# AliBahri94/GM3D

Hardware: AMD Instinct MI355X
Metric: point-clouds/sec pretrain step (N=1024,G=64) (higher is better)
Workload: dtype bf16

## Files before the change

### gm3d_amd/csrc/gemm_ws.hip

```cpp
#include "mfma.hpp"

namespace gm3d {

__device__ __forceinline__ void ws_wait_vm(int n) {
#define GM3D_WS_CASE(N_) case N_: asm volatile("s_waitcnt vmcnt(%0)" ::"n"(N_) : "memory"); break;
    switch (n) {
        GM3D_WS_CASE(0) GM3D_WS_CASE(4) GM3D_WS_CASE(8) GM3D_WS_CASE(12) GM3D_WS_CASE(16) GM3D_WS_CASE(24) GM3D_WS_CASE(32)
        GM3D_WS_CASE(36) GM3D_WS_CASE(48)
        default: asm volatile("s_waitcnt vmcnt(0)" ::: "memory"); break;
    }
#undef GM3D_WS_CASE
}

struct WsBn {
    const bf16_t* T;
    const float* scale;
    const float* shift;
    float* partial;
    int ldt;
    float slope;
};

constexpr int ws_depth(int ppl, int tile, int stage) {
    int d = 48 / ppl < 4 ? 48 / ppl : 4;
    while (d > 1 && (d + 1) * tile + stage > 152 * 1024) --d;
    return d;
}

template <int KT, int NW, int NL, int EPI, int TM>
__global__ __launch_bounds__(64 * (NW + NL)) void gemm_tn_ws_kernel(const bf16_t* __restrict__ A, const bf16_t* __restrict__ W,
                                                                     const float* __restrict__ bias, bf16_t* __restrict__ C, int M, int N,
                                                                     int lda, int ldw, int ldc, int tiles_n, bf16_t* __restrict__ P,
                                                                     uint8_t* __restrict__ ARG, int ldp, int bias_after_pool, WsBn bn,
                                                                     int Kreal, int pool16) {
    extern __shared__ __attribute__((aligned(16))) unsigned char wsm[];
    constexpr int BN = 32 * NW, NIMG = BN / 64 > 0 ? (BN + 63) / 64 : 1;
    constexpr int HALF = KT * 4096;
    constexpr int TILE = TM * HALF;
    constexpr int NP = TM * 4 * KT;
    constexpr int PPL = NP / NL;
    constexpr int STAGE = TM * NIMG * 4096;
    constexpr int DEPTH = ws_depth(PPL, TILE, STAGE);
    constexpr int NT = DEPTH + 1;
    static_assert(NP % NL == 0 && PPL <= 48, "loader split");
    unsigned char* stage = wsm + NT * TILE;
    const int tid = threadIdx.x, lane = tid & 63, w = __builtin_amdgcn_readfirstlane(tid >> 6);
    const int r = lane & 31, hh = lane >> 5;
    const int logical = xcd_tile(blockIdx.x, gridDim.x);
    const int tile_n = logical % tiles_n, first = logical / tiles_n, stride = gridDim.x / tiles_n;
    const int tiles_m = (M + 32 * TM - 1) / (32 * TM);
    const int nmine = first < tiles_m ? (tiles_m - first + stride - 1) / stride : 0;
    const int n0 = tile_n * BN;
    const unsigned lds0 = lds_addr(wsm);

    if (w >= NW) {
        const int lw = w - NW, prow = lane >> 3, pslot = lane & 7;
        auto issue = [&](int i) {
            const int m0 = (first + i * stride) * (32 * TM);
            const unsigned base = lds0 + (i % NT) * TILE;
#pragma unroll
            for (int q = 0; q < PPL; ++q) {
                const int p = lw * PPL + q, t = p / (4 * KT), pp = p - t * (4 * KT), kt = pp >> 2, row = 8 * (pp & 3) + prow;
                const int gr = m0 + 32 * t + row;
                const int am = gr < M ? gr : M - 1;
                int col = 64 * kt + ((pslot ^ swz(row)) << 3);
                col = col < Kreal ? col : 0;
                glds16(A + (size_t)am * lda + col, base + 1024 * p);
            }
        };
        for (int d = 0; d < DEPTH && d < nmine; ++d) issue(d);
        for (int i = 0; i < nmine; ++i) {
            if (i + DEPTH < nmine) issue(i + DEPTH);
            const int ahead = nmine - 1 - i < DEPTH ? nmine - 1 - i : DEPTH;
            ws_wait_vm(ahead * PPL);
            __builtin_amdgcn_s_barrier();
            __builtin_amdgcn_s_barrier();
        }
        return;
    }

    bf16x8 wreg[KT][4];
    {
        const bf16_t* wp = W + (size_t)(n0 + 32 * w + r) * ldw + 8 * hh;
#pragma unroll
        for (int kt = 0; kt < KT; ++kt)
#pragma unroll
            for (int s = 0; s < 4; ++s) {
                if (64 * kt + 16 * s + 8 * hh < Kreal) wreg[kt][s] = *reinterpret_cast<const bf16x8*>(wp + 64 * kt + 16 * s);
                else
#pragma unroll
                    for (int e = 0; e < 8; ++e) wreg[kt][s][e] = (bf16_t)0.0f;
            }
    }
    float bq[4][4];
#pragma unroll
    for (int q = 0; q < 4; ++q)
#pragma unroll
        for (int e = 0; e < 4; ++e) bq[q][e] = (EPI != 3 && bias) ? bias[n0 + 32 * w + 8 * q + 4 * hh + e] : 0.f;
    const float bcol = (EPI == 3 && bias) ? bias[n0 + 32 * w + r] : 0.f;
    const bool bias_in_tile = EPI != 3 || !bias_after_pool;
    float bn_a[4][4], bn_b[4][4];
    if (EPI == 4 || EPI == 5) {
#pragma unroll
        for (int q = 0; q < 4; ++q)
#pragma unroll
            for (int e = 0; e < 4; ++e) {
                const int col = n0 + 32 * w + 8 * q + 4 * hh + e;
                bn_a[q][e] = EPI == 4 ? bn.scale[col] : 0.f;
                bn_b[q][e] = EPI == 4 ? bn.shift[col] : 0.f;
            }
    }
    constexpr int CTHREADS = 64 * NW;

    for (int i = 0; i < nmine; ++i) {
        const int m0 = (first + i * stride) * (32 * TM);
        float tq[TM][4][4];
        if (EPI == 4 || EPI == 5) {
            typedef const __attribute__((address_space(4))) unsigned int* sptr_t;
#pragma unroll
            for (int t = 0; t < TM; ++t) {
                const size_t trow = pool16 ? (size_t)2 * ((m0 >> 5) + t) : (size_t)((m0 >> 5) + t);
                sptr_t tp = (sptr_t)(const void*)(bn.T + trow * bn.ldt + n0 + 32 * w);
                unsigned tw[16];
#pragma unroll
                for (int j = 0; j < 16; ++j) tw[j] = tp[j];
                if (pool16) {
                    sptr_t tp2 = (sptr_t)(const void*)(bn.T + (trow + 1) * bn.ldt + n0 + 32 * w);
                    unsigned tw2[16];
#pragma unroll
                    for (int j = 0; j < 16; ++j) tw2[j] = tp2[j];
                    if (r & 16) {
#pragma unroll
                        for (int j = 0; j < 16; ++j) tw[j] = tw2[j];
                    }
                }
#pragma unroll
                for (int q = 0; q < 4; ++q)
#pragma unroll
                    for (int e2 = 0; e2 < 2; ++e2) {
                        const unsigned u = hh ? tw[4 * q + 2 + e2] : tw[4 * q + e2];
                        tq[t][q][2 * e2] = __builtin_bit_cast(float, u << 16);
                        tq[t][q][2 * e2 + 1] = __builtin_bit_cast(float, u & 0xffff0000u);
                    }
            }
        }
        __builtin_amdgcn_s_barrier();
        const unsigned char* as = wsm + (i % NT) * TILE;
        f32x16 acc[TM];
#pragma unroll
        for (int t = 0; t < TM; ++t)
#pragma unroll
            for (int g = 0; g < 16; ++g) acc[t][g] = 0.f;
#pragma unroll
        for (int kt = 0; kt < KT; ++kt) {
            bf16x8 fa[TM][4];
#pragma unroll
            for (int t = 0; t < TM; ++t)
#pragma unroll
                for (int s = 0; s < 4; ++s) fa[t][s] = *reinterpret_cast<const bf16x8*>(as + t * HALF + kt * 4096 + swz_off(r, 2 * s + hh));
#pragma unroll
            for (int s = 0; s < 4; ++s)
#pragma unroll
                for (int t = 0; t < TM; ++t)
                    acc[t] = EPI == 3 ? mfma_bf16(fa[t][s], wreg[kt][s], acc[t])
                                      : mfma_bf16(wreg[kt][s], fa[t][s], acc[t]);
        }
        if (EPI == 3 && !C) __builtin_amdgcn_s_barrier();
        if (EPI == 3) {
            unsigned short rowbits[TM][16];
#pragma unroll
            for (int t = 0; t < TM; ++t) {
                unsigned best = 0, best2 = 0;
#pragma unroll
                for (int g = 0; g < 16; ++g) {
                    const bf16_t o = (bf16_t)(acc[t][g] + (bias_in_tile ? bcol : 0.f));
                    rowbits[t][g] = __builtin_bit_cast(unsigned short, o);
                    unsigned u = (unsigned)rowbits[t][g] << 16;
                    u = u == 0x80000000u ? 0u : u;
                    const unsigned k = (u ^ (unsigned)(((int)u >> 31) | (int)0x80000000)) & 0xffff0000u;
                    const unsigned key = k | (unsigned)(31 - (8 * (g >> 2) + 4 * hh + (g & 3)));
                    if (pool16 && g >= 8) best2 = key > best2 ? key : best2;
                    else best = key > best ? key : best;
                }
                {
                    const unsigned other = (unsigned)__shfl_xor((int)best, 32);
                    best = other > best ? other : best;
                    const unsigned other2 = (unsigned)__shfl_xor((int)best2, 32);
                    best2 = other2 > best2 ? other2 : best2;
                }
                if (hh == 0 && m0 + 32 * t < M) {
                    const unsigned k = best & 0xffff0000u;
                    const unsigned u = (k & 0x80000000u) ? (k & 0x7fff0000u) : (~k & 0xffff0000u);
                    float v = __builtin_bit_cast(float, u);
                    if (bias_after_pool) v += bcol;
                    if (!pool16) {
                        const size_t o = (size_t)((m0 >> 5) + t) * ldp + n0 + 32 * w + r;
                        P[o] = (bf16_t)v;
                        ARG[o] = (uint8_t)(31u - (best & 0xffu));
                    } else {
                        const size_t o = (size_t)((m0 >> 4) + 2 * t) * ldp + n0 + 32 * w + r;
                        P[o] = (bf16_t)v;
                        ARG[o] = (uint8_t)(31u - (best & 0xffu));
                        if (m0 + 32 * t + 16 < M) {
                            const unsigned k2 = best2 & 0xffff0000u;
                            const unsigned u2 = (k2 & 0x80000000u) ? (k2 & 0x7fff0000u) : (~k2 & 0xffff0000u);
                            float v2 = __builtin_bit_cast(float, u2);
                            if (bias_after_pool) v2 += bcol;
                            P[o + ldp] = (bf16_t)v2;
                            ARG[o + ldp] = (uint8_t)(15u - (best2 & 0xffu));
                        }
                    }
                }
            }
            if (!C) continue;
            const int ch = (((32 * w) & 63) + r) >> 3, sub = 2 * (r & 7);
#pragma unroll
            for (int t = 0; t < TM; ++t) {
                unsigned char* img = stage + (t * NIMG + ((32 * w) >> 6)) * 4096;
#pragma unroll
                for (int g = 0; g < 16; ++g) {
                    const int row = 8 * (g >> 2) + 4 * hh + (g & 3);
                    *reinterpret_cast<unsigned short*>(img + swz_off(row, ch) + sub) = rowbits[t][g];
                }
            }
        } else {
            const int cbase = ((32 * w) & 63) >> 3;
#pragma unroll
            for (int t = 0; t < TM; ++t) {
                unsigned char* img = stage + (t * NIMG + ((32 * w) >> 6)) * 4096;
#pragma unroll
                for (int q = 0; q < 4; ++q) {
                    bf16x4 pk;
#pragma unroll
                    for (int e = 0; e < 4; ++e) {
                        pk[e] = (bf16_t)(acc[t][4 * q + e] + bq[q][e]);
                        if (EPI == 4) {
                            const float h = ((float)pk[e] + tq[t][q][e]) * bn_a[q][e] + bn_b[q][e];
                            pk[e] = (bf16_t)(h > 0.f ? h : bn.slope * h);
                        }
                        if (EPI == 5) {
                            const float y = (float)pk[e] + tq[t][q][e];
                            bn_a[q][e] += y;
                            bn_b[q][e] += y * y;
                        }
                    }
                    *reinterpret_cast<bf16x4*>(img + swz_off(r, cbase + q) + 8 * hh) = pk;
                }
            }
        }
        asm volatile("s_waitcnt lgkmcnt(0)" ::: "memory");
        __builtin_amdgcn_s_barrier();
        {
            constexpr int CH = BN / 8;
#pragma unroll
            for (int c0 = 0; c0 < 32 * TM * CH; c0 += CTHREADS) {
                const int c = c0 + tid;
                if (c < 32 * TM * CH) {
                    const int row = c / CH, chunk = c - row * CH;
                    if (m0 + row < M) {
                        const uint4 raw = *reinterpret_cast<const uint4*>(stage + ((row >> 5) * NIMG + (chunk >> 3)) * 4096 + swz_off(row & 31, chunk & 7));
                        *reinterpret_cast<uint4*>(C + (size_t)(m0 + row) * ldc + n0 + 8 * chunk) = raw;
                    }
                }
            }
        }
    }
    if (EPI == 5) {
#pragma unroll
        for (int q = 0; q < 4; ++q)
#pragma unroll
            for (int e = 0; e < 4; ++e) {
#pragma unroll
                for (int m = 1; m < 32; m <<= 1) {
                    bn_a[q][e] += __shfl_xor(bn_a[q][e], m);
                    bn_b[q][e] += __shfl_xor(bn_b[q][e], m);
                }
                if (r == 0) {
                    const int col = n0 + 32 * w + 8 * q + 4 * hh + e;
                    bn.partial[(size_t)first * 2 * N + col] = bn_a[q][e];
                    bn.partial[(size_t)first * 2 * N + N + col] = bn_b[q][e];
                }
            }
    }
}

}

using gm3d::ws_depth;

static int ws_grid(int tiles_m, int tiles_n, size_t lds) {
    long long want = (long long)tiles_m * tiles_n;
    const int cap = 2 * lds <= 160 * 1024 ? 512 : 256;
    int g = want < cap ? (int)want : cap;
    g = (g + 7) / 8 * 8;
    while (g % tiles_n) g += 8;
    return g;
}

static int ws_launch(const void* A, const void* W, const float* bias, void* C, void* P, uint8_t* ARG, int M, int N, int K, int lda,
                     int ldw, int ldc, int ldp, int bias_after_pool, gm3d_stream_t stream, int bn_mode = 0, gm3d::WsBn bn = gm3d::WsBn(),
                     int pool16 = 0) {
    using namespace gm3d;
    if (!A || !W || (!C && !P) || M < 0 || N < 1 || K < 1) return GM3D_EINVAL;
    if (P && (!ARG || M % (pool16 ? 16 : 32) || ldp % 8 || ldp < N || ((size_t)ARG & 7) || ((size_t)P & 15))) return GM3D_EINVAL;
    if (K % 8 || K > 512 || lda % 8 || ldw % 8 || lda < K || ldw < K || (C && (ldc % 8 || ldc < N))) return GM3D_EUNSUPPORTED;
    if (((size_t)A | (size_t)W | (size_t)C) & 15) return GM3D_EUNSUPPORTED;
    if (M == 0) return GM3D_OK;
#define GM3D_WS_LAUNCH(KT, NW, NL, EPI, TM)                                                                               \
    {                                                                                                                    \
        constexpr int TILE_ = TM * KT * 4096, STAGE_ = TM * ((32 * NW + 63) / 64) * 4096;                                \
        constexpr int DEPTH_ = ws_depth(TM * 4 * KT / NL, TILE_, STAGE_);                                                \
        const size_t lds = (size_t)(DEPTH_ + 1) * TILE_ + STAGE_;                                                        \
        const int tiles_m = (M + 32 * TM - 1) / (32 * TM);                                                               \
        const int tiles_n = N / (32 * NW), grid = ws_grid(tiles_m, tiles_n, lds);                                        \
        return launch_lds<gemm_tn_ws_kernel<KT, NW, NL, EPI, TM>>(dim3(grid), dim3(64 * (NW + NL)), lds, stream, (const bf16_t*)A, \
                                                                  (const bf16_t*)W, bias, (bf16_t*)C, M, N, lda, ldw, ldc, tiles_n, \
                                                                  (bf16_t*)P, ARG, ldp, bias_after_pool, bn, K, pool16);        \
    }
    if (P) {
        if (K == 128 && N == 256) GM3D_WS_LAUNCH(2, 8, 1, 3, 1)
        if (K == 512 && N == 384) GM3D_WS_LAUNCH(8, 6, 2, 3, 1)
        if (K == 512 && N == 96) GM3D_WS_LAUNCH(8, 3, 2, 3, 1)
        return GM3D_EUNSUPPORTED;
    }
    if (bn_mode) {
        if (M % 32 || !bn.T || bn.ldt % 4 || bn.ldt < N || ((size_t)bn.T & 7)) return GM3D_EINVAL;
        if (K == 256 && N == 512 && bn_mode == 4) GM3D_WS_LAUNCH(4, 8, 1, 4, 1)
        if (K == 256 && N == 512 && bn_mode == 5) GM3D_WS_LAUNCH(4, 8, 1, 5, 1)
        return GM3D_EUNSUPPORTED;
    }
    if (K == 256 && N == 512) GM3D_WS_LAUNCH(4, 8, 1, 0, 1)
    if (K == 512 && N == 256) GM3D_WS_LAUNCH(8, 4, 2, 0, 1)
    if (K == 384 && N == 512) GM3D_WS_LAUNCH(6, 8, 2, 0, 1)
    if (K == 256 && N == 128) GM3D_WS_LAUNCH(4, 4, 1, 0, 1)
    if (K == 128 && N == 256) GM3D_WS_LAUNCH(2, 8, 1, 0, 1)
    if (K == 512 && N == 384) GM3D_WS_LAUNCH(8, 6, 2, 0, 1)
    if (K == 96 && N == 288) GM3D_WS_LAUNCH(2, 9, 1, 0, 1)
    if (K == 96 && N == 96) GM3D_WS_LAUNCH(2, 3, 1, 0, 1)
    if (K == 96 && N == 512) GM3D_WS_LAUNCH(2, 8, 1, 0, 1)
    if (K == 96 && N == 192) GM3D_WS_LAUNCH(2, 6, 1, 0, 1)
    if (K == 192 && N == 96) GM3D_WS_LAUNCH(3, 3, 1, 0, 1)
    if (K == 96 && N == 384) GM3D_WS_LAUNCH(2, 6, 1, 0, 1)
    if (K == 384 && N == 96) GM3D_WS_LAUNCH(6, 3, 1, 0, 1)
    if (K == 288 && N == 96) GM3D_WS_LAUNCH(5, 3, 1, 0, 1)
#undef GM3D_WS_LAUNCH
    return GM3D_EUNSUPPORTED;
}

extern "C" int gm3d_gemm_tn_bf16_ws(const void* A, const void* W, const float* bias, void* C, int M, int N, int K, int lda, int ldw,
                                    int ldc, gm3d_stream_t stream) {
    if (!C) return GM3D_EINVAL;
    return ws_launch(A, W, bias, C, nullptr, nullptr, M, N, K, lda, ldw, ldc, 0, 0, stream);
}

extern "C" int gm3d_gemm_tn_bf16_ws_pool(const void* A, const void* W, const float* bias, void* C, void* P, uint8_t* arg, int M, int N,
                                         int K, int lda, int ldw, int ldc, int ldp, int bias_after_pool, gm3d_stream_t stream) {
    if (!P || !arg) return GM3D_EINVAL;
    return ws_launch(A, W, bias, C, P, arg, M, N, K, lda, ldw, ldc, ldp, bias_after_pool, stream);
}

extern "C" int gm3d_gemm_tn_bf16_ws_poolg(const void* A, const void* W, const float* bias, void* C, void* P, uint8_t* arg, int M, int N,
                                          int K, int lda, int ldw, int ldc, int ldp, int bias_after_pool, int group_rows,
                                          gm3d_stream_t stream) {
    if (!P || !arg || (group_rows != 16 && group_rows != 32)) return GM3D_EINVAL;
    return ws_launch(A, W, bias, C, P, arg, M, N, K, lda, ldw, ldc, ldp, bias_after_pool, stream, 0, gm3d::WsBn(), group_rows == 16);
}

extern "C" int gm3d_gemm_tn_bf16_ws_bn_apply(const void* A, const void* W, const void* T, const float* scale, const float* shift, float slope,
                                             void* C, int M, int N, int K, int lda, int ldw, int ldt, int ldc, gm3d_stream_t stream) {
    if (!C || !T || !scale || !shift) return GM3D_EINVAL;
    gm3d::WsBn bn;
    bn.T = (const gm3d::bf16_t*)T; bn.scale = scale; bn.shift = shift; bn.partial = nullptr; bn.ldt = ldt; bn.slope = slope;
    return ws_launch(A, W, nullptr, C, nullptr, nullptr, M, N, K, lda, ldw, ldc, 0, 0, stream, 4, bn);
}

extern "C" int gm3d_gemm_tn_bf16_ws_bn_stats(const void* A, const void* W, const void* T, void* C, float* partial, int M, int N, int K,
                                             int lda, int ldw, int ldt, int ldc, gm3d_stream_t stream) {
    if (!C || !T || !partial) return GM3D_EINVAL;
    gm3d::WsBn bn;
    bn.T = (const gm3d::bf16_t*)T; bn.scale = nullptr; bn.shift = nullptr; bn.partial = partial; bn.ldt = ldt; bn.slope = 0.f;
    return ws_launch(A, W, nullptr, C, nullptr, nullptr, M, N, K, lda, ldw, ldc, 0, 0, stream, 5, bn);
}

extern "C" int gm3d_gemm_tn_bf16_ws_bn_apply_g(const void* A, const void* W, const void* T, const float* scale, const float* shift, float slope,
                                               void* C, int M, int N, int K, int lda, int ldw, int ldt, int ldc, int group_rows,
                                               gm3d_stream_t stream) {
    if (!C || !T || !scale || !shift || (group_rows != 16 && group_rows != 32)) return GM3D_EINVAL;
    gm3d::WsBn bn;
    bn.T = (const gm3d::bf16_t*)T; bn.scale = scale; bn.shift = shift; bn.partial = nullptr; bn.ldt = ldt; bn.slope = slope;
    return ws_launch(A, W, nullptr, C, nullptr, nullptr, M, N, K, lda, ldw, ldc, 0, 0, stream, 4, bn, group_rows == 16);
}

extern "C" int gm3d_gemm_tn_bf16_ws_bn_stats_g(const void* A, const void* W, const void* T, void* C, float* partial, int M, int N, int K,
                                               int lda, int ldw, int ldt, int ldc, int group_rows, gm3d_stream_t stream) {
    if (!C || !T || !partial || (group_rows != 16 && group_rows != 32)) return GM3D_EINVAL;
    gm3d::WsBn bn;
    bn.T = (const gm3d::bf16_t*)T; bn.scale = nullptr; bn.shift = nullptr; bn.partial = partial; bn.ldt = ldt; bn.slope = 0.f;
    return ws_launch(A, W, nullptr, C, nullptr, nullptr, M, N, K, lda, ldw, ldc, 0, 0, stream, 5, bn, group_rows == 16);
}

extern "C" int gm3d_gemm_ws_stats_rows(int M, int N, int K) {
    if (!(K == 256 && N == 512) || M % 32 || M < 32) return 0;
    constexpr int KT = 4, NW = 8, NL = 1;
    constexpr int TILE_ = KT * 4096, STAGE_ = ((32 * NW + 63) / 64) * 4096;
    const size_t lds = (size_t)(ws_depth(4 * KT / NL, TILE_, STAGE_) + 1) * TILE_ + STAGE_;
    const int tiles_n = N / (32 * NW);
    return ws_grid(M / 32, tiles_n, lds) / tiles_n;
}

extern "C" int gm3d_gemm_ws_supported(int N, int K, int pool) {
    if (pool) return (K == 128 && N == 256) || (K == 512 && N == 384) || (K == 512 && N == 96);
    return (K == 256 && N == 512) || (K == 512 && N == 256) || (K == 384 && N == 512) || (K == 256 && N == 128) ||
           (K == 128 && N == 256) || (K == 512 && N == 384) || (K == 96 && (N == 288 || N == 96 || N == 384 || N == 192 || N == 512)) || (K == 384 && N == 96) ||
           (K == 288 && N == 96) || (K == 192 && N == 96);
}
```

Before: 17150.

## Double-buffer epilogue staging and overlap tile stores with next tile's MFMAs

Adds a second LDS staging buffer so each tile's global stores are interleaved into the next tile's MFMA loop rather than run after a barrier. It also prefetches the BN residual (T) rows for the next tile, software-pipelines the A-fragment LDS reads one k-step ahead, and picks pipeline depth and LDS size through a new config function with a register-budget check. The aim is to hide epilogue store latency and per-tile load latency behind compute. The cost is extra LDS, which can reduce pipeline depth, plus higher register pressure and more complex scheduling.

```diff
diff --git a/gm3d_amd/csrc/gemm_ws.hip b/gm3d_amd/csrc/gemm_ws.hip
--- a/gm3d_amd/csrc/gemm_ws.hip
+++ b/gm3d_amd/csrc/gemm_ws.hip
@@ -21,10 +21,28 @@
     float slope;
 };
 
-constexpr int ws_depth(int ppl, int tile, int stage) {
+constexpr int ws_depth1(int ppl, int tile, int stage) {
     int d = 48 / ppl < 4 ? 48 / ppl : 4;
     while (d > 1 && (d + 1) * tile + stage > 152 * 1024) --d;
     return d;
+}
+constexpr int ws_depth(int ppl, int tile, int stage) {
+    int d = ws_depth1(ppl, tile, stage);
+    const bool two = 2 * ((d + 1) * tile + stage) <= 160 * 1024;
+    while (d > 1 && ((d + 1) * tile + 2 * stage > 152 * 1024 || (two && 2 * ((d + 1) * tile + 2 * stage) > 160 * 1024))) --d;
+    return d;
+}
+struct WsCfg {
+    bool pipe;
+    int depth, lds;
+};
+constexpr WsCfg ws_cfg(int kt, int nw, int nl, int epi, int tm) {
+    const int tile = tm * kt * 4096, stage = tm * ((32 * nw + 63) / 64) * 4096, ppl = tm * 4 * kt / nl;
+    const int d1 = ws_depth1(ppl, tile, stage), d = ws_depth(ppl, tile, stage);
+    const int budget = 512 / ((nw + nl + 3) / 4) / 8 * 8;
+    const bool regs = 16 * kt + 16 * tm + 16 * tm + (epi >= 4 ? 32 : 16) + 32 <= budget;
+    const bool pipe = regs && (d >= 2 || d == d1);
+    return pipe ? WsCfg{true, d, (d + 1) * tile + 2 * stage} : WsCfg{false, d1, (d1 + 1) * tile + stage};
 }
 
 template <int KT, int NW, int NL, int EPI, int TM>
@@ -40,7 +58,10 @@
     constexpr int NP = TM * 4 * KT;
     constexpr int PPL = NP / NL;
     constexpr int STAGE = TM * NIMG * 4096;
-    constexpr int DEPTH = ws_depth(PPL, TILE, STAGE);
+    constexpr WsCfg CFG = ws_cfg(KT, NW, NL, EPI, TM);
+    constexpr bool PIPE = CFG.pipe;
+    constexpr int DEPTH = CFG.depth;
+    static_assert(CFG.lds == (DEPTH + 1) * TILE + (PIPE ? 2 : 1) * STAGE, "LDS layout");
     constexpr int NT = DEPTH + 1;
     static_assert(NP % NL == 0 && PPL <= 48, "loader split");
     unsigned char* stage = wsm + NT * TILE;
@@ -96,7 +117,7 @@
 #pragma unroll
     for (int q = 0; q < 4; ++q)
 #pragma unroll
-        for (int e = 0; e < 4; ++e) bq[q][e] = (EPI != 3 && bias) ? bias[n0 + 32 * w + 8 * q + 4 * hh + e] : 0.f;
+        for (int e = 0; e < 4; ++e) bq[q][e] = (EPI == 0 && bias) ? bias[n0 + 32 * w + 8 * q + 4 * hh + e] : 0.f;
     const float bcol = (EPI == 3 && bias) ? bias[n0 + 32 * w + r] : 0.f;
     const bool bias_in_tile = EPI != 3 || !bias_after_pool;
     float bn_a[4][4], bn_b[4][4];
@@ -111,39 +132,47 @@
             }
     }
     constexpr int CTHREADS = 64 * NW;
-
+    constexpr int CH = BN / 8, NCHK = 32 * TM * CH / CTHREADS, NMF = 4 * KT, SLICE = NMF / NCHK;
+    static_assert(NCHK * CTHREADS == 32 * TM * CH && SLICE >= 2, "row-store split");
+    static_assert(CTHREADS == 16 * CH, "row-store split");
+    const int row0 = tid / CH, chunk = tid - row0 * CH;
+    const int soff = (chunk >> 3) * 4096 + swz_off(row0, chunk & 7);
+    const unsigned goff = (unsigned)(row0 * ldc + n0 + 8 * chunk);
+    auto chunk_read = [&](const unsigned char* sg, int j) {
+        return *reinterpret_cast<const uint4*>(sg + soff + (j & 1) * 2048 + (j >> 1) * NIMG * 4096);
+    };
+    auto chunk_store = [&](int mt, int mlim, int j, const uint4& raw) {
+        if (mt + 16 * j + row0 < mlim) *reinterpret_cast<uint4*>(C + (size_t)(mt + 16 * j) * ldc + goff) = raw;
+    };
+    unsigned tn[TM][16], tn2[TM][16];
+#pragma unroll
+    for (int t = 0; t < TM; ++t)
+#pragma unroll
+        for (int j = 0; j < 16; ++j) tn[t][j] = tn2[t][j] = 0u;
+    auto fetch_t = [&](int mt) {
+        typedef const __attribute__((address_space(4))) unsigned int* sptr_t;
+#pragma unroll
+        for (int t = 0; t < TM; ++t) {
+            const size_t trow = pool16 ? (size_t)2 * ((mt >> 5) + t) : (size_t)((mt >> 5) + t);
+            sptr_t tp = (sptr_t)(const void*)(bn.T + trow * bn.ldt + n0 + 32 * w);
+#pragma unroll
+            for (int j = 0; j < 16; ++j) tn[t][j] = tp[j];
+            if (pool16) {
+                sptr_t tp2 = (sptr_t)(const void*)(bn.T + (trow + 1) * bn.ldt + n0 + 32 * w);
+#pragma unroll
+                for (int j = 0; j < 16; ++j) tn2[t][j] = tp2[j];
+            }
+        }
+    };
+    if ((EPI == 4 || EPI == 5) && nmine > 0) fetch_t(first * (32 * TM));
+
+    int mprev = 0;
     for (int i = 0; i < nmine; ++i) {
         const int m0 = (first + i * stride) * (32 * TM);
-        float tq[TM][4][4];
-        if (EPI == 4 || EPI == 5) {
-            typedef const __attribute__((address_space(4))) unsigned int* sptr_t;
-#pragma unroll
-            for (int t = 0; t < TM; ++t) {
-                const size_t trow = pool16 ? (size_t)2 * ((m0 >> 5) + t) : (size_t)((m0 >> 5) + t);
-                sptr_t tp = (sptr_t)(const void*)(bn.T + trow * bn.ldt + n0 + 32 * w);
-                unsigned tw[16];
-#pragma unroll
-                for (int j = 0; j < 16; ++j) tw[j] = tp[j];
-                if (pool16) {
-                    sptr_t tp2 = (sptr_t)(const void*)(bn.T + (trow + 1) * bn.ldt + n0 + 32 * w);
-                    unsigned tw2[16];
-#pragma unroll
-                    for (int j = 0; j < 16; ++j) tw2[j] = tp2[j];
-                    if (r & 16) {
-#pragma unroll
-                        for (int j = 0; j < 16; ++j) tw[j] = tw2[j];
-                    }
-                }
-#pragma unroll
-                for (int q = 0; q < 4; ++q)
-#pragma unroll
-                    for (int e2 = 0; e2 < 2; ++e2) {
-                        const unsigned u = hh ? tw[4 * q + 2 + e2] : tw[4 * q + e2];
-                        tq[t][q][2 * e2] = __builtin_bit_cast(float, u << 16);
-                        tq[t][q][2 * e2 + 1] = __builtin_bit_cast(float, u & 0xffff0000u);
-                    }
-            }
-        }
+        unsigned char* sg = stage + (PIPE ? (i & 1) * STAGE : 0);
+        const unsigned char* sgp = stage + ((i & 1) ^ 1) * STAGE;
+        const bool drainp = PIPE && i > 0 && C;
+        const int mlim = drainp ? M : 0;
         __builtin_amdgcn_s_barrier();
         const unsigned char* as = wsm + (i % NT) * TILE;
         f32x16 acc[TM];
@@ -151,19 +180,32 @@
         for (int t = 0; t < TM; ++t)
 #pragma unroll
             for (int g = 0; g < 16; ++g) acc[t][g] = 0.f;
+        bf16x8 fa[TM][4];
+        uint4 raw[NCHK];
+#pragma unroll
+        for (int t = 0; t < TM; ++t)
+#pragma unroll
+            for (int s = 0; s < 4; ++s) fa[t][s] = *reinterpret_cast<const bf16x8*>(as + t * HALF + swz_off(r, 2 * s + hh));
 #pragma unroll
         for (int kt = 0; kt < KT; ++kt) {
-            bf16x8 fa[TM][4];
-#pragma unroll
-            for (int t = 0; t < TM; ++t)
-#pragma unroll
-                for (int s = 0; s < 4; ++s) fa[t][s] = *reinterpret_cast<const bf16x8*>(as + t * HALF + kt * 4096 + swz_off(r, 2 * s + hh));
-#pragma unroll
-            for (int s = 0; s < 4; ++s)
-#pragma unroll
-                for (int t = 0; t < TM; ++t)
+#pragma unroll
+            for (int s = 0; s < 4; ++s) {
+                if (PIPE) {
+#pragma unroll
+                    for (int j = 0; j < NCHK; ++j) {
+                        if (4 * kt + s == 1 + j * SLICE && drainp) raw[j] = chunk_read(sgp, j);
+                        if (4 * kt + s == 2 + j * SLICE) chunk_store(mprev, mlim, j, raw[j]);
+                    }
+                }
+#pragma unroll
+                for (int t = 0; t < TM; ++t) {
+                    __builtin_amdgcn_sched_barrier(0);
                     acc[t] = EPI == 3 ? mfma_bf16(fa[t][s], wreg[kt][s], acc[t])
                                       : mfma_bf16(wreg[kt][s], fa[t][s], acc[t]);
+                    if (kt + 1 < KT)
+                        fa[t][s] = *reinterpret_cast<const bf16x8*>(as + t * HALF + (kt + 1) * 4096 + swz_off(r, 2 * s + hh));
+                }
+            }
         }
         if (EPI == 3 && !C) __builtin_amdgcn_s_barrier();
         if (EPI == 3) {
@@ -216,7 +258,7 @@
             const int ch = (((32 * w) & 63) + r) >> 3, sub = 2 * (r & 7);
 #pragma unroll
             for (int t = 0; t < TM; ++t) {
-                unsigned char* img = stage + (t * NIMG + ((32 * w) >> 6)) * 4096;
+                unsigned char* img = sg + (t * NIMG + ((32 * w) >> 6)) * 4096;
 #pragma unroll
                 for (int g = 0; g < 16; ++g) {
                     const int row = 8 * (g >> 2) + 4 * hh + (g & 3);
@@ -225,45 +267,56 @@
             }
         } else {
             const int cbase = ((32 * w) & 63) >> 3;
+            int rs = r;
+            asm volatile("" : "+v"(rs));
 #pragma unroll
             for (int t = 0; t < TM; ++t) {
-                unsigned char* img = stage + (t * NIMG + ((32 * w) >> 6)) * 4096;
+                unsigned char* img = sg + (t * NIMG + ((32 * w) >> 6)) * 4096;
 #pragma unroll
                 for (int q = 0; q < 4; ++q) {
                     bf16x4 pk;
+                    float tq[4];
+                    if (EPI == 4 || EPI == 5) {
+#pragma unroll
+                        for (int e2 = 0; e2 < 2; ++e2) {
+                            const int j = 4 * q + e2;
+                            const unsigned lo = (pool16 && (r & 16)) ? tn2[t][j] : tn[t][j];
+                            const unsigned hi = (pool16 && (r & 16)) ? tn2[t][j + 2] : tn[t][j + 2];
+                            const unsigned u = hh ? hi : lo;
+                            tq[2 * e2] = __builtin_bit_cast(float, u << 16);
+                            tq[2 * e2 + 1] = __builtin_bit_cast(float, u & 0xffff0000u);
+                        }
+                    }
 #pragma unroll
                     for (int e = 0; e < 4; ++e) {
                         pk[e] = (bf16_t)(acc[t][4 * q + e] + bq[q][e]);
                         if (EPI == 4) {
-                            const float h = ((float)pk[e] + tq[t][q][e]) * bn_a[q][e] + bn_b[q][e];
+                            const float h = ((float)pk[e] + tq[e]) * bn_a[q][e] + bn_b[q][e];
                             pk[e] = (bf16_t)(h > 0.f ? h : bn.slope * h);
                         }
                         if (EPI == 5) {
-                            const float y = (float)pk[e] + tq[t][q][e];
+                            const float y = (float)pk[e] + tq[e];
                             bn_a[q][e] += y;
-                            bn_b[q][e] += y * y;
+                            bn_b[q][e] = __builtin_fmaf(y, y, bn_b[q][e]);
                         }
                     }
-                    *reinterpret_cast<bf16x4*>(img + swz_off(r, cbase + q) + 8 * hh) = pk;
+                    *reinterpret_cast<bf16x4*>(img + swz_off(rs, cbase + q) + 8 * hh) = pk;
                 }
             }
         }
         asm volatile("s_waitcnt lgkmcnt(0)" ::: "memory");
         __builtin_amdgcn_s_barrier();
-        {
-            constexpr int CH = BN / 8;
-#pragma unroll
-            for (int c0 = 0; c0 < 32 * TM * CH; c0 += CTHREADS) {
-                const int c = c0 + tid;
-                if (c < 32 * TM * CH) {
-                    const int row = c / CH, chunk = c - row * CH;
-                    if (m0 + row < M) {
-                        const uint4 raw = *reinterpret_cast<const uint4*>(stage + ((row >> 5) * NIMG + (chunk >> 3)) * 4096 + swz_off(row & 31, chunk & 7));
-                        *reinterpret_cast<uint4*>(C + (size_t)(m0 + row) * ldc + n0 + 8 * chunk) = raw;
-                    }
-                }
-            }
+        if ((EPI == 4 || EPI == 5) && i + 1 < nmine) fetch_t(m0 + stride * (32 * TM));
+        if (!PIPE) {
+#pragma unroll
+            for (int j = 0; j < NCHK; ++j) chunk_store(m0, M, j, chunk_read(sg, j));
         }
+        mprev = m0;
+    }
+    if (PIPE && nmine > 0 && (EPI != 3 || C)) {
+        const unsigned char* sgl = stage + ((nmine - 1) & 1) * STAGE;
+#pragma unroll
+        for (int j = 0; j < NCHK; ++j) chunk_store(mprev, M, j, chunk_read(sgl, j));
     }
     if (EPI == 5) {
 #pragma unroll
@@ -286,7 +339,7 @@
 
 }
 
-using gm3d::ws_depth;
+using gm3d::ws_depth1;
 
 static int ws_grid(int tiles_m, int tiles_n, size_t lds) {
     long long want = (long long)tiles_m * tiles_n;
@@ -309,8 +362,12 @@
 #define GM3D_WS_LAUNCH(KT, NW, NL, EPI, TM)                                                                               \
     {                                                                                                                    \
         constexpr int TILE_ = TM * KT * 4096, STAGE_ = TM * ((32 * NW + 63) / 64) * 4096;                                \
-        constexpr int DEPTH_ = ws_depth(TM * 4 * KT / NL, TILE_, STAGE_);                                                \
-        const size_t lds = (size_t)(DEPTH_ + 1) * TILE_ + STAGE_;                                                        \
+        constexpr int LDS_ = gm3d::ws_cfg(KT, NW, NL, EPI, TM).lds;                                                      \
+                     \
+        static_assert((2 * LDS_ <= 160 * 1024) ==                                                                        \
+                          (2 * ((ws_depth1(TM * 4 * KT / NL, TILE_, STAGE_) + 1) * TILE_ + STAGE_) <= 160 * 1024),       \
+                      "ws_grid residency");                                                                              \
+        const size_t lds = LDS_;                                                                                         \
         const int tiles_m = (M + 32 * TM - 1) / (32 * TM);                                                               \
         const int tiles_n = N / (32 * NW), grid = ws_grid(tiles_m, tiles_n, lds);                                        \
         return launch_lds<gemm_tn_ws_kernel<KT, NW, NL, EPI, TM>>(dim3(grid), dim3(64 * (NW + NL)), lds, stream, (const bf16_t*)A, \
@@ -402,8 +459,7 @@
 extern "C" int gm3d_gemm_ws_stats_rows(int M, int N, int K) {
     if (!(K == 256 && N == 512) || M % 32 || M < 32) return 0;
     constexpr int KT = 4, NW = 8, NL = 1;
-    constexpr int TILE_ = KT * 4096, STAGE_ = ((32 * NW + 63) / 64) * 4096;
-    const size_t lds = (size_t)(ws_depth(4 * KT / NL, TILE_, STAGE_) + 1) * TILE_ + STAGE_;
+    const size_t lds = gm3d::ws_cfg(KT, NW, NL, 5, 1).lds;
     const int tiles_n = N / (32 * NW);
     return ws_grid(M / 32, tiles_n, lds) / tiles_n;
 }
```

After: 17150 (median of 2 runs). Within noise of the previous version (+0.0%).
